# alevar/tiebrush

Hardware: AMD Instinct MI355X
Metric: input alignment records/sec collapsed (tiebrush) + bases/sec covered (tiecov) (higher is better)
Workload: dtype int64; 1 GPU; c3: 64 synthetic sorted BAMs x 5000000 100bp reads per GPU, --clip collapse + tiecov -c -j of the result; records_per_gpu=320000000, groups_out=25086541, parallelism=files-per-rank x1, ranks_seen=1, resident=SoA in HBM before the timed region, contexts=3

## Files before the change

### tiebrush_amd/csrc/collapse.hip

```cpp
#include <stdlib.h>

#include <chrono>

#include "dev_common.hpp"
#include "rx_w64.hpp"
#include "scan_op.hpp"
#include "strategy.hpp"
#include "tbk_internal.h"
#include "wgroup.h"

namespace {

struct EffKey {
  uint32_t khi_h, khi_l;
  int32_t kend;
  uint32_t flag_cnt;
};
struct EffOp {
  __device__ __forceinline__ EffKey operator()(const EffKey& a, const EffKey& b) const {
    uint64_t ak = ((uint64_t)a.khi_h << 32) | a.khi_l, bk = ((uint64_t)b.khi_h << 32) | b.khi_l;
    bool take_b = (b.flag_cnt >> 31) || bk > ak || (bk == ak && b.kend > a.kend);
    EffKey r;
    r.khi_h = take_b ? b.khi_h : a.khi_h;
    r.khi_l = take_b ? b.khi_l : a.khi_l;
    r.kend = take_b ? b.kend : a.kend;
    r.flag_cnt = ((a.flag_cnt | b.flag_cnt) & 0x80000000u) | ((a.flag_cnt + b.flag_cnt) & 0x7FFFFFFFu);
// ... 2359 lines not shown
  cnt[o] = cig_off[rep[o] + 1] - c0;
  cfirst[o] = c0;
}
__device__ __forceinline__ uint32_t g2c_key_ops(uint64_t k1) {
  const uint32_t shape = (uint32_t)k1;
  return shape == 0x80000000u ? 1u : ((shape >> 30) == 3u ? 3u : 0u);
}
__global__ void g2c_count_key_k(uint32_t ng, const uint64_t* __restrict__ key, const uint32_t* __restrict__ rep, const uint32_t* __restrict__ cig_off,
                                uint32_t* __restrict__ cnt, uint32_t* __restrict__ cfirst) {
  uint32_t o = blockIdx.x * blockDim.x + threadIdx.x;
  if (o >= ng) return;
  uint32_t n = g2c_key_ops(key[2 * (size_t)o + 1]);
  if (n == 0) {
    const uint32_t c0 = cig_off[rep[o]];
    n = cig_off[rep[o] + 1] - c0;
    cfirst[o] = c0;
  }
  cnt[o] = n;
}
struct G2cPrep {
  int32_t *start, *end, *yi;
  uint32_t *jcnt, *ridx;
  unsigned long long* sums;
};
__global__ __launch_bounds__(256) void g2c_gather_key_k(uint32_t ng, const uint64_t* __restrict__ key, const double* __restrict__ yc,
                                                        const int64_t* __restrict__ yx, const uint32_t* __restrict__ cfirst,
                                                        const uint32_t* __restrict__ cnt, const uint32_t* __restrict__ cig,
                                                        const uint32_t* __restrict__ ooff, uint32_t total, int32_t* __restrict__ o_tid,
                                                        int32_t* __restrict__ o_pos, uint8_t* __restrict__ o_strand, double* __restrict__ o_yc,
                                                        int64_t* __restrict__ o_yx, uint32_t* __restrict__ o_cig_off, uint32_t* __restrict__ o_cig,
                                                        G2cPrep P) {
  unsigned long long mb = 0, ay = 0, nji = 0;
  uint32_t eb = 0;
  for (uint32_t o = blockIdx.x * blockDim.x + threadIdx.x; o < ng; o += gridDim.x * blockDim.x) {
    const uint64_t k0 = key[2 * (size_t)o], k1 = key[2 * (size_t)o + 1];
    const int32_t tidv = (int32_t)(uint32_t)(k0 >> 33) - 1, posv = (int32_t)(uint32_t)((k0 >> 2) & 0x7FFFFFFFull) - 1;
    o_tid[o] = tidv;
    o_pos[o] = posv;
    const uint32_t sc = (uint32_t)k0 & 3u;
    o_strand[o] = sc == 0u ? (uint8_t)'+' : (sc == 1u ? (uint8_t)'-' : (uint8_t)'.');
    const double y0 = (double)(float)yc[o];
    o_yc[o] = y0;
    o_yx[o] = yx[o];
    const uint32_t d = ooff[o];
    o_cig_off[o] = d;
    if (o + 1 == ng) o_cig_off[ng] = total;
    const uint32_t shape = (uint32_t)k1, span = (uint32_t)(k1 >> 32);
    int l, nex = 0;
    if (shape == 0x80000000u) {
      o_cig[d] = (span << 4) | C_M;
      l = (int)span;
      nex = 1;
      mb += span;
    } else if ((shape >> 30) == 3u) {
      const uint32_t a = (shape >> 20) & 0x3FFu, g = shape & 0xFFFFFu;
      o_cig[d] = (a << 4) | C_M;
      o_cig[d + 1] = (g << 4) | C_N;
      o_cig[d + 2] = ((span - a - g) << 4) | C_M;
      l = (int)span;
      nex = 2;
      mb += span - g;
    } else {
      const uint32_t c0 = cfirst[o], n = cnt[o];
      l = walk_exons(posv, cig + c0, n, [](int, int) {}, &nex);
      for (uint32_t k = 0; k < n; ++k) {
        const uint32_t w = cig[c0 + k];
        o_cig[d + k] = w;
        const uint32_t op = cig_op(w);
        if (op == C_M)
          mb += cig_len(w);
        else if (op != C_I && op != C_D && op != C_N && op != C_S)
          eb |= TBK_DERR_FATALOP;
      }
      if (n >= 256) eb |= TBK_DERR_NCIGAR;
    }
    double y = y0;
    if (!(y == rint(y)) || !(fabs(y) < 1073741824.0)) {
      eb |= TBK_DERR_FRACTIONAL;
      y = 0.0;
    } else {
      ay += (unsigned long long)fabs(y);
    }
    P.ridx[o] = o;
    P.yi[o] = (int32_t)y;
    P.start[o] = posv + 1;
    P.end[o] = posv + l;
    P.jcnt[o] = (uint32_t)(nex - 1);
    nji += (unsigned long long)(nex - 1);
  }
  __shared__ unsigned long long red_mb[4], red_ay[4], red_nj[4];
  __shared__ uint32_t red_e[4];
  mb = wave_sum(mb);
  ay = wave_sum(ay);
  nji = wave_sum(nji);
#pragma unroll
  for (int dd = 32; dd >= 1; dd >>= 1) eb |= __shfl_xor(eb, dd, 64);
  if (lane_id() == 0) {
    red_mb[threadIdx.x >> 6] = mb;
    red_ay[threadIdx.x >> 6] = ay;
    red_nj[threadIdx.x >> 6] = nji;
    red_e[threadIdx.x >> 6] = eb;
  }
  __syncthreads();
  if (threadIdx.x == 0) {
    for (int q = 1; q < 4; ++q) {
      mb += red_mb[q];
      ay += red_ay[q];
      nji += red_nj[q];
      eb |= red_e[q];
    }
    if (mb) atomicAdd(&P.sums[0], mb);
    if (ay) atomicAdd(&P.sums[1], ay);
    if (eb) atomicOr(&P.sums[2], (unsigned long long)eb);
    if (nji) atomicAdd(&P.sums[3], nji);
  }
}
__global__ void g2c_gather_k(uint32_t ng, const uint32_t* __restrict__ rep, const double* __restrict__ yc, const int64_t* __restrict__ yx,
                             const int32_t* __restrict__ tid, const int32_t* __restrict__ pos, const uint8_t* __restrict__ strand,
                             const uint32_t* __restrict__ cfirst, const uint32_t* __restrict__ cnt, const uint32_t* __restrict__ cig,
                             const uint32_t* __restrict__ ooff, uint32_t total, int32_t* __restrict__ o_tid, int32_t* __restrict__ o_pos,
                             uint8_t* __restrict__ o_strand, double* __restrict__ o_yc, int64_t* __restrict__ o_yx,
                             uint32_t* __restrict__ o_cig_off, uint32_t* __restrict__ o_cig) {
  uint32_t o = blockIdx.x * blockDim.x + threadIdx.x;
  if (o >= ng) return;
  uint32_t r = rep[o];
  o_tid[o] = tid[r];
  o_pos[o] = pos[r];
  o_strand[o] = strand[r];
  o_yc[o] = (double)(float)yc[o];
  o_yx[o] = yx[o];
  uint32_t d = ooff[o];
  o_cig_off[o] = d;
  if (o + 1 == ng) o_cig_off[ng] = total;
  const uint32_t c0 = cfirst[o], n = cnt[o];
  for (uint32_t k = 0; k < n; ++k) o_cig[d + k] = cig[c0 + k];
}
}

// ... 17 lines not shown
int tbk_cov_view_build(tbk_ctx* ctx, const int32_t* r_tid, const int32_t* r_pos, const uint8_t* r_strand, const uint32_t* r_cig_off,
                       const uint32_t* r_cig, const uint32_t* g_rep, const double* g_yc, const int64_t* g_yx, uint32_t ng, tbk_cov_in* view,
                       const uint64_t* g_key) {
  memset(view, 0, sizeof(*view));
  view->mem = TBK_MEM_DEVICE;
  ctx->view_prep.valid = false;
  if (ng == 0) return 0;
  uint32_t* cnt = ws_alloc<uint32_t>(ctx, ng);
  uint32_t* ooff = ws_alloc<uint32_t>(ctx, ng);
  uint32_t* cfirst = ws_alloc<uint32_t>(ctx, ng);
  if (!cfirst) return TBK_ENOMEM;
  const uint32_t B = 256;
  if (g_key)
    TBK_LAUNCH(ctx, "g2c_count", g2c_count_key_k, cdiv(ng, B), B, 0, ng, g_key, g_rep, r_cig_off, cnt, cfirst);
  else
    TBK_LAUNCH(ctx, "g2c_count", g2c_count_k, cdiv(ng, B), B, 0, ng, g_rep, r_cig_off, cnt, cfirst);
  TBK_TRY(tbk_exscan_u32(ctx, cnt, ooff, ng, ctx->d_scalars + 20));
  TBK_HIP(hipMemcpyAsync(ctx->h_scalars + 20, ctx->d_scalars + 20, sizeof(uint64_t), hipMemcpyDeviceToHost, ctx->stream));
  TBK_HIP(hipStreamSynchronize(ctx->stream));
  const uint64_t total = ctx->h_scalars[20];
  if (total >= (1ull << 32)) return TBK_E2BIG;
  auto al = [](size_t x) { return (x + 255) & ~(size_t)255; };
  size_t need = al((size_t)ng * 4) * 2 + al(ng) + al((size_t)ng * 8) * 2 + al((size_t)(ng + 1) * 4) + al((size_t)total * 4 + 4) +
                (g_key ? al((size_t)ng * 4) * 5 : 0);
  if (need > ctx->d_view_cap) {
    if (ctx->d_view) (void)hipFree(ctx->d_view);
    ctx->d_view = nullptr;
    ctx->d_view_cap = 0;
    size_t cap = need + need / 4;
    TBK_HIP(hipMalloc((void**)&ctx->d_view, cap));
    ctx->d_view_cap = cap;
  }
  char* p = ctx->d_view;
  auto take = [&](size_t bytes) {
    char* r = p;
    p += al(bytes);
    return r;
  };
  int32_t* o_tid = (int32_t*)take((size_t)ng * 4);
  int32_t* o_pos = (int32_t*)take((size_t)ng * 4);
  uint8_t* o_strand = (uint8_t*)take(ng);
  double* o_yc = (double*)take((size_t)ng * 8);
  int64_t* o_yx = (int64_t*)take((size_t)ng * 8);
  uint32_t* o_cig_off = (uint32_t*)take((size_t)(ng + 1) * 4);
  uint32_t* o_cig = (uint32_t*)take((size_t)total * 4 + 4);
  G2cPrep P{};
  if (g_key) {
    P.start = (int32_t*)take((size_t)ng * 4);
    P.end = (int32_t*)take((size_t)ng * 4);
    P.yi = (int32_t*)take((size_t)ng * 4);
    P.jcnt = (uint32_t*)take((size_t)ng * 4);
    P.ridx = (uint32_t*)take((size_t)ng * 4);
    P.sums = (unsigned long long*)(ctx->d_scalars + 24);
    TBK_HIP(hipMemsetAsync(P.sums, 0, 4 * sizeof(uint64_t), ctx->stream));
    TBK_LAUNCH(ctx, "g2c_gather", g2c_gather_key_k, (cdiv(ng, B) < 4096u ? cdiv(ng, B) : 4096u), B, 0, ng, g_key, g_yc, g_yx, cfirst, cnt, r_cig, ooff,
               (uint32_t)total, o_tid, o_pos, o_strand, o_yc, o_yx, o_cig_off, o_cig, P);
    TBK_HIP(hipMemcpyAsync(ctx->h_scalars + 24, ctx->d_scalars + 24, 4 * sizeof(uint64_t), hipMemcpyDeviceToHost, ctx->stream));
  } else
    TBK_LAUNCH(ctx, "g2c_gather", g2c_gather_k, cdiv(ng, B), B, 0, ng, g_rep, g_yc, g_yx, r_tid, r_pos, r_strand, cfirst, cnt, r_cig, ooff,
               (uint32_t)total, o_tid, o_pos, o_strand, o_yc, o_yx, o_cig_off, o_cig);
  TBK_HIP(hipStreamSynchronize(ctx->stream));
  TBK_TRY(tbk_check_launch(ctx, "groups_to_cov_in"));
  view->n_records = ng;
  view->n_cigar_ops = (uint32_t)total;
  view->tid = o_tid;
  view->pos = o_pos;
  view->flag = nullptr;
  view->cig_off = o_cig_off;
  view->cig = o_cig;
  view->yc = o_yc;
  view->strand = o_strand;
  view->yx = o_yx;
  if (g_key) {
    auto& V = ctx->view_prep;
    V.cig = o_cig;
    V.n = ng;
    V.start = P.start;
    V.end = P.end;
    V.yi = P.yi;
    V.jcnt = P.jcnt;
    V.ridx = P.ridx;
    V.n_bases = ctx->h_scalars[24];
    V.sum_abs = ctx->h_scalars[25];
    V.err = (uint32_t)ctx->h_scalars[26];
    V.n_junc = ctx->h_scalars[27];
    V.valid = true;
  }
  return 0;
}
```

### tiebrush_amd/csrc/cov.hip

```cpp
#include <thread>

#include "dev_common.hpp"
#include "scan_op.hpp"
#include "tbk_internal.h"

namespace {

constexpr int COV_W = 8192;
constexpr int COV_NT = 256;
constexpr int COV_PER = COV_W / COV_NT;

struct SegMax {
  int32_t mx;
  uint32_t flag;
};
struct SegMaxOp {
  __device__ __forceinline__ SegMax operator()(const SegMax& a, const SegMax& b) const {
    SegMax r;
    r.mx = b.flag ? b.mx : (a.mx > b.mx ? a.mx : b.mx);
    r.flag = a.flag | b.flag;
    return r;
  }
};

// ... 109 lines not shown
};
struct BundleStore {
  CovArrays A;
  uint32_t m;
  uint64_t* nb_out;
  uint32_t* err;
  __device__ __forceinline__ void operator()(uint32_t j, const SegMax& v, const SegMax& inc, const SegMax&, uint32_t head, uint32_t before,
                                             const int2& a) const {
    const int32_t t = a.y, st = a.x;
    if (!v.flag && st < A.start[j - 1]) atomicOr(err, TBK_DERR_UNSORTED);
    const uint32_t b = before + head - 1u;
    A.bhead[j] = head;
    A.bid[j] = b;
    if (head) {
      A.b_tid[b] = t;
      A.b_start[b] = st;
    }
    const bool last = j + 1 == m;
    if (last || A.tid[j + 1] != t || A.start[j + 1] > inc.mx) A.b_end[b] = inc.mx;
    if (last) *nb_out = (uint64_t)b + 1u;
  }
};

struct CbAgg {
  int32_t first_tid, last_tid;
  int32_t mx;
  uint32_t whole;
};
struct CbOp {
  __device__ __forceinline__ CbAgg operator()(const CbAgg& a, const CbAgg& b) const {
    if (b.last_tid == INT32_MIN) return a;
    if (a.last_tid == INT32_MIN) return b;
    CbAgg r;
    r.first_tid = a.first_tid;
    r.last_tid = b.last_tid;
    const bool joins = b.whole && b.first_tid == a.last_tid;
    r.mx = joins ? (a.mx > b.mx ? a.mx : b.mx) : b.mx;
    r.whole = joins ? a.whole : 0u;
    return r;
  }
};
constexpr uint32_t CB_NT = 256, CB_ROWS = 4, CB_TILE = CB_NT * 4 * CB_ROWS;
__device__ __forceinline__ void cb_load4(const int32_t* __restrict__ a, uint64_t i, uint32_t m, int32_t fill, int32_t v[4]) {
  if (i + 3 < m) {
    const int4 q = *reinterpret_cast<const int4*>(a + i);
    v[0] = q.x, v[1] = q.y, v[2] = q.z, v[3] = q.w;
  } else {
#pragma unroll
    for (int e = 0; e < 4; ++e) v[e] = i + e < m ? a[i + e] : fill;
  }
}
template <class T, class Op>
__device__ __forceinline__ T wave_incl_scan_op(T v, Op op) {
#pragma unroll
  for (int d = 1; d < 64; d <<= 1) {
    const T o = shfl_up_t(v, d);
    if ((int)lane_id() >= d) v = op(o, v);
  }
  return v;
}
__device__ __forceinline__ void cb_put(uint64_t* p, uint64_t v) { __hip_atomic_store(p, v, __ATOMIC_RELAXED, __HIP_MEMORY_SCOPE_AGENT); }
__device__ __forceinline__ uint64_t cb_get(const uint64_t* p) { return __hip_atomic_load(p, __ATOMIC_RELAXED, __HIP_MEMORY_SCOPE_AGENT); }
__device__ __forceinline__ uint4 cb_get4(const uint4* p) {
  const uint64_t a = cb_get(reinterpret_cast<const uint64_t*>(p)), b = cb_get(reinterpret_cast<const uint64_t*>(p) + 1);
  return make_uint4((uint32_t)a, (uint32_t)(a >> 32), (uint32_t)b, (uint32_t)(b >> 32));
}
__device__ __forceinline__ bool cb_last_block(uint32_t* __restrict__ done) {
  __shared__ uint32_t s_last;
  if (threadIdx.x == 0) {
    __builtin_amdgcn_s_waitcnt(TBK_WAIT_VMCNT0);
    __asm__ volatile("" ::: "memory");
    s_last = atomicAdd(done, 1u) == gridDim.x - 1u ? 1u : 0u;
  }
  __syncthreads();
  return s_last != 0u;
}
template <uint32_t NT>
__device__ __forceinline__ void cb_spine_block(uint4* __restrict__ part, uint32_t ntiles, CbAgg* wl ) {
  const CbOp op{};
  const CbAgg none{0, INT32_MIN, INT32_MIN, 1u};
  auto un = [](const uint4& v) { return CbAgg{(int32_t)v.x, (int32_t)v.y, (int32_t)v.z, v.w}; };
  auto pk = [](const CbAgg& a) { return make_uint4((uint32_t)a.first_tid, (uint32_t)a.last_tid, (uint32_t)a.mx, a.whole); };
  const uint4 none4 = pk(none);
  const uint32_t per = (ntiles + NT - 1u) / NT, i0 = threadIdx.x * per, i1 = i0 + per < ntiles ? i0 + per : ntiles;
  CbAgg a = none;
  for (uint32_t q0 = i0; q0 < i1; q0 += 8u) {
    uint4 v8[8];
#pragma unroll
    for (uint32_t u = 0; u < 8u; ++u) v8[u] = q0 + u < i1 ? cb_get4(part + q0 + u) : none4;
#pragma unroll
    for (uint32_t u = 0; u < 8u; ++u) a = op(a, un(v8[u]));
  }
  const CbAgg inc = wave_incl_scan_op(a, op);
  if (lane_id() == 63) wl[threadIdx.x >> 6] = inc;
  CbAgg run = shfl_up_t(inc, 1);
  __syncthreads();
  {
    CbAgg acc = none;
    const uint32_t wv = threadIdx.x >> 6;
    for (uint32_t q = 0; q < wv; ++q) acc = op(acc, wl[q]);
    run = lane_id() == 0 ? acc : op(acc, run);
  }
  for (uint32_t q0 = i0; q0 < i1; q0 += 8u) {
    uint4 v8[8];
#pragma unroll
    for (uint32_t u = 0; u < 8u; ++u) v8[u] = q0 + u < i1 ? cb_get4(part + q0 + u) : none4;
#pragma unroll
    for (uint32_t u = 0; u < 8u; ++u) {
      if (q0 + u < i1) part[q0 + u] = pk(run);
      run = op(run, un(v8[u]));
    }
  }
}
__global__ __launch_bounds__(CB_NT) void cb_agg_k(uint32_t m, const int32_t* __restrict__ tid, const int32_t* __restrict__ end, uint4* __restrict__ part,
                                                  uint32_t* __restrict__ done) {
  constexpr uint32_t NWV = CB_NT / 64;
  __shared__ CbAgg wl[CB_ROWS * NWV];
  const CbOp op{};
  const CbAgg none{0, INT32_MIN, INT32_MIN, 1u};
  int32_t t4[CB_ROWS][4], e4[CB_ROWS][4];
#pragma unroll
  for (uint32_t r = 0; r < CB_ROWS; ++r) {
    const uint64_t i = (uint64_t)blockIdx.x * CB_TILE + ((uint64_t)r * CB_NT + threadIdx.x) * 4u;
    cb_load4(tid, i, m, 0, t4[r]);
    cb_load4(end, i, m, 0, e4[r]);
  }
#pragma unroll
  for (uint32_t r = 0; r < CB_ROWS; ++r) {
    const uint64_t i = (uint64_t)blockIdx.x * CB_TILE + ((uint64_t)r * CB_NT + threadIdx.x) * 4u;
    CbAgg a = none;
#pragma unroll
    for (int e = 0; e < 4; ++e)
      if (i + e < m) a = op(a, CbAgg{t4[r][e], t4[r][e], e4[r][e], 1u});
    a = wave_incl_scan_op(a, op);
    if (lane_id() == 63) wl[r * NWV + (threadIdx.x >> 6)] = a;
  }
  __syncthreads();
  if (threadIdx.x == 0) {
    CbAgg run = none;
#pragma unroll
    for (uint32_t q = 0; q < CB_ROWS * NWV; ++q) run = op(run, wl[q]);
    uint64_t* o = reinterpret_cast<uint64_t*>(part + blockIdx.x);
    cb_put(o, (uint64_t)(uint32_t)run.first_tid | ((uint64_t)(uint32_t)run.last_tid << 32));
    cb_put(o + 1, (uint64_t)(uint32_t)run.mx | ((uint64_t)run.whole << 32));
  }
  if (cb_last_block(done)) cb_spine_block<CB_NT>(part, gridDim.x, wl);
}
template <bool EMIT>
__global__ __launch_bounds__(CB_NT) void cb_heads_k(uint32_t m, CovArrays A, const uint4* __restrict__ part, uint32_t* __restrict__ hcnt,
                                                    const uint32_t* __restrict__ hbase, uint64_t* __restrict__ nb_out, uint32_t* __restrict__ err) {
  __shared__ CbAgg sm[CB_NT / 64];
  __shared__ uint32_t smu[8];
  const CbOp op{};
  const CbAgg none{0, INT32_MIN, INT32_MIN, 1u};
  const uint4 pv = part[blockIdx.x];
  CbAgg run{(int32_t)pv.x, (int32_t)pv.y, (int32_t)pv.z, pv.w};
  uint32_t heads_tile = 0, hrun = EMIT ? hbase[blockIdx.x] : 0u;
  bool bad = false;
#pragma unroll
  for (uint32_t r = 0; r < CB_ROWS; ++r) {
    const uint64_t i = (uint64_t)blockIdx.x * CB_TILE + ((uint64_t)r * CB_NT + threadIdx.x) * 4u;
    int32_t t4[4], s4[4], e4[4];
    cb_load4(A.tid, i, m, 0, t4);
    cb_load4(A.start, i, m, 0, s4);
    cb_load4(A.end, i, m, 0, e4);
    CbAgg a = none;
#pragma unroll
// ... 1459 lines not shown
    TBK_LAUNCH(ctx, "junc_write", junc_write_k, cdiv(nj, B), B, 0, nj, A, sb.hi, sb.lo, sb.val, head, hoff, in->yc, out->cap_junctions,
               out->j_tid, out->j_start, out->j_end, out->j_strand, out->j_val);
  }
  TBK_HIP(hipMemcpyAsync(ctx->h_scalars + 9, sc + 9, sizeof(uint64_t), hipMemcpyDeviceToHost, ctx->stream));
  TBK_HIP(hipStreamSynchronize(ctx->stream));
  *nju_out = (uint32_t)ctx->h_scalars[9];
  return tbk_check_launch(ctx, "junctions");
}

struct JuncSide {
  TbkWorker* w = nullptr;
  bool th = false;
  int rc = 0;
  int join() {
    if (th) {
      w->wait();
      th = false;
    }
    return rc;
  }
  ~JuncSide() { (void)join(); }
};

static int cov_intervals_lean(tbk_ctx* ctx, const tbk_cov_in* in, tbk_cov_out* out, CovArrays A, uint32_t m, bool all_valid, uint64_t sum_abs) {
  const uint32_t B = 256;
  uint64_t* sc = ctx->d_scalars;
  const uint32_t cbt = cdiv(m, CB_TILE);
  uint4* cpart = ws_alloc<uint4>(ctx, cbt);
  uint32_t* hcnt = ws_alloc<uint32_t>(ctx, cbt);
  uint32_t* hbase = ws_alloc<uint32_t>(ctx, cbt);
  long long* xsum = ws_alloc<long long>(ctx, cbt);
  long long* xbase = ws_alloc<long long>(ctx, cbt);
  ClChunks L;
  L.base = ws_alloc<uint32_t>(ctx, cbt);
  L.cnt = ws_alloc<uint32_t>(ctx, cbt);
  L.tbase = ws_alloc<uint32_t>(ctx, cbt);
  L.j = ws_alloc<uint32_t>(ctx, m);
  L.cs = ws_alloc<uint64_t>(ctx, m);
  ClTiles T;
  uint64_t cap64 = (uint64_t)m / 8u > (1ull << 20) ? (uint64_t)m / 8u : (1ull << 20);
  if (ctx->dbg.cov_tile_cap) cap64 = ctx->dbg.cov_tile_cap;
  T.cap = (uint32_t)cap64;
  T.first = ws_alloc<uint32_t>(ctx, (size_t)T.cap + 1);
  T.tb = ws_alloc<uint32_t>(ctx, (size_t)T.cap + 1);
  T.cnt = ws_alloc<uint32_t>(ctx, (size_t)T.cap + 1);
  if (!cpart || !hcnt || !hbase || !xsum || !xbase || !L.base || !L.cnt || !L.tbase || !L.j || !L.cs || !T.first || !T.tb || !T.cnt) return TBK_ENOMEM;
  TBK_HIP(hipMemsetAsync(T.cnt, 0, ((size_t)T.cap + 1) * 4, ctx->stream));
  uint32_t* done = (uint32_t*)(sc + 16);
  TBK_HIP(hipMemsetAsync(done, 0, sizeof(uint64_t), ctx->stream));
  TBK_LAUNCH(ctx, "cov_bundles", cb_agg_k, cbt, CB_NT, 0, m, A.tid, A.end, cpart, done);
  TBK_LAUNCH(ctx, "cov_bundles", cl_heads_k<false>, cbt, CB_NT, 0, m, A, cpart, hcnt, xsum, (const uint32_t*)nullptr, (const long long*)nullptr, in->cig_off,
             in->cig, T, L, sc, ctx->d_err, done + 1, hbase, xbase);
  TBK_LAUNCH(ctx, "cov_place", cl_heads_k<true>, cbt, CB_NT, 0, m, A, cpart, hcnt, xsum, hbase, xbase, in->cig_off, in->cig, T, L, sc, ctx->d_err,
             (uint32_t*)nullptr, (uint32_t*)nullptr, (long long*)nullptr);
  uint32_t eb = 0;
  TBK_TRY(tbk_sync_err(ctx, &eb));
  if (eb) return tbk_derr_to_status(ctx, eb);
  if (ctx->h_scalars[CL_SC_REFUSED]) return 1;
  const uint32_t nb = (uint32_t)ctx->h_scalars[CL_SC_NB];
  const uint64_t S = ctx->h_scalars[CL_SC_S], nspill = ctx->h_scalars[CL_SC_NSPILL];
  const uint32_t nsl = (uint32_t)ctx->h_scalars[CL_SC_NSL];
  out->span_bases = S;
  const uint32_t ntiles = (uint32_t)((S + COV_W - 1) / COV_W);
  if (nspill >= (1ull << 32)) return TBK_E2BIG;
  const uint64_t cp_cap64 = 2ull * ((uint64_t)in->n_cigar_ops + nspill) + nb + ntiles + 16;
  if (cp_cap64 >= (1ull << 32)) return TBK_E2BIG;
  const uint32_t cp_cap = (uint32_t)cp_cap64;
  uint32_t* tile_off = ws_alloc<uint32_t>(ctx, (size_t)ntiles + 1);
  uint32_t* tile_fill = ws_alloc<uint32_t>(ctx, (size_t)ntiles + 1);
  uint32_t* sp_seg = ws_alloc<uint32_t>(ctx, nspill + 1);
  uint32_t* sp_rec = ws_alloc<uint32_t>(ctx, nspill + 1);
  uint64_t* cp_pos = ws_alloc<uint64_t>(ctx, cp_cap);
  double* cp_val = ws_alloc<double>(ctx, cp_cap);
  uint32_t* tile_cp_base = ws_alloc<uint32_t>(ctx, ntiles);
  uint32_t* tile_cp_cnt = ws_alloc<uint32_t>(ctx, ntiles);
  uint32_t* icnt = ws_alloc<uint32_t>(ctx, ntiles);
// ... 96 lines not shown
  out->n_bases = ctx->h_scalars[0];
  const uint64_t sum_abs = ctx->h_scalars[1];
  const bool integral = !fractional && !sample_mode && sum_abs < (1ull << 52);
  const uint64_t nj_known = prepared ? V.n_junc : (want_j ? ctx->h_scalars[14] : ~0ull);
  if (m == 0) return 0;
  if (want_j && want_cov && m >= COV_SIDE_MIN) {
    tbk_ctx* jc = tbk_side_ctx(ctx);
    if (jc) {
      const size_t hint = (size_t)m * 8 + (size_t)in->n_cigar_ops * 64 + ((size_t)4 << 20);
      if (!ctx->side_worker) ctx->side_worker = new TbkWorker();
      side.w = ctx->side_worker;
      side.th = true;
      side.w->post([&side, jc, hint, m, &A, in, jcnt, out, integral, nj_known, &nj, &nju]() {
        side.rc = tbk_side_begin(jc, hint);
        if (side.rc == 0) side.rc = junc_branch(jc, m, A, in, jcnt, out, integral, nj_known, &nj, &nju);
        tbk_side_end(jc);
      });
    }
  }

  bool lean_done = false;
  if (want_cov && !fractional && !sample_mode && !ctx->dbg.cov_legacy && !ctx->dbg.cov_bundle_scan) {
    const size_t ws_mark = ctx->ws_off;
    const int lrc = cov_intervals_lean(ctx, in, out, A, m, all_valid, sum_abs);
    if (lrc < 0) return lrc;
    lean_done = lrc == 0;
    if (!lean_done) {
      if (ctx->ws_overflow.empty()) ctx->ws_off = ws_mark;
      TBK_HIP(hipMemsetAsync(sc + 3, 0, 11 * sizeof(uint64_t), ctx->stream));
    }
  }
  if (!lean_done) {
  {
    if (ctx->dbg.cov_bundle_scan) {
      BundleLoad ld{A.tid, A.end};
      BundleAux ax{A.tid, A.start};
      BundleHead hd{};
      BundleStore st{A, m, sc + 3, ctx->d_err};
      SegMax ident{INT32_MIN, 0u};
      TBK_TRY((scan_two_run<4, SegMax, SegMaxOp, uint32_t, SoPlusU32, BundleLoad, BundleAux, BundleHead, BundleStore>(ctx, "cov_bundles", m, ld, ax, hd, st, SegMaxOp{}, ident,
                                                                                                          SoPlusU32{}, 0u)));
    } else {
      const uint32_t cbt = cdiv(m, CB_TILE);
      uint4* cpart = ws_alloc<uint4>(ctx, cbt);
      uint32_t* hcnt = ws_alloc<uint32_t>(ctx, cbt);
      uint32_t* hbase = ws_alloc<uint32_t>(ctx, cbt);
      if (!cpart || !hcnt || !hbase) return TBK_ENOMEM;
// ... 143 lines not shown
```

### tiebrush_amd/csrc/tbk_api.hip

```cpp
#include <sys/mman.h>

#include <algorithm>
#include <chrono>
#include <mutex>
#include <vector>
#include <new>

#include "tbk_internal.h"

namespace {
std::mutex g_reg_m;
struct RegEntry {
  void* p;
  int users;
};
std::vector<RegEntry> g_reg;
}

static void release_registered(tbk_ctx* ctx) {
  if (ctx->registered.empty()) return;
  (void)hipStreamSynchronize(ctx->stream);
  const auto r0 = std::chrono::steady_clock::now();
  struct RP {
    tbk_ctx* c;
// ... 431 lines not shown
    if (end == std::string::npos) end = s.size();
    const std::string kv = s.substr(at, end - at);
    at = end + 1;
    const size_t eq = kv.find('=');
    const std::string k = kv.substr(0, eq), v = eq == std::string::npos ? std::string("1") : kv.substr(eq + 1);
    const unsigned long long u = strtoull(v.c_str(), nullptr, 0);
    const bool on = v != "0";
    if (k == "path") out->path = v == "sort" ? 1 : (v == "window" ? 2 : 0);
    else if (k == "raw") out->raw = on ? 1 : 0;
    else if (k == "sort") out->sort = v == "radix" ? 1 : (v == "runs" ? 2 : 0);
    else if (k == "scan") out->scan = v == "lookback" ? 1 : (v == "3pass" ? 2 : 0);
    else if (k == "hash_mask") out->hash_mask = (uint32_t)u;
    else if (k == "qhash_mask") out->qhash_mask = u;
    else if (k == "yd_wave_min") out->yd_wave_min = (uint32_t)u;
    else if (k == "yd_bgrid") out->yd_bgrid = (uint32_t)u;
    else if (k == "yd_radix") out->yd_radix = on;
    else if (k == "yd_literal") out->yd_literal = on;
    else if (k == "yd_own_arena") out->yd_own_arena = on;
    else if (k == "wg_dense_verify") out->wg_dense_verify = on;
    else if (k == "wg_rank_merge") out->wg_rank_merge = on;
    else if (k == "cov_legacy") out->cov_legacy = on;
    else if (k == "cov_bundle_scan") out->cov_bundle_scan = on;
    else if (k == "cov_prep") out->cov_prep = on;
    else if (k == "cov_tile_cap") out->cov_tile_cap = u;
    else if (k == "junc_radix") out->junc_radix = on;
    else if (k == "no_junc_agg") out->no_junc_agg = on;
    else if (k == "jh_cap") out->jh_cap = (uint32_t)u;
    else if (k == "index_chain") out->index_chain = on;
    else if (k == "no_register") out->no_register = on;
    else if (k == "phases") out->phases = on;
    else if (k == "no_bounce") out->no_bounce = on;
    else if (k == "fmt_slice") out->fmt_slice = u;
  }
}

extern "C" {

int tbk_abi_version(void) { return TBK_ABI_VERSION; }

int tbk_set_debug(tbk_ctx* ctx, const char* spec) {
  if (!ctx) return TBK_EINVAL;
  tbk_debug_parse(spec, &ctx->dbg);
  if (ctx->yd_ctx) ctx->yd_ctx->dbg = ctx->dbg;
  if (ctx->side_ctx) ctx->side_ctx->dbg = ctx->dbg;
  return 0;
}
// ... 494 lines not shown
```

### tiebrush_amd/csrc/tbk_internal.h

```cpp
#pragma once
#include <hip/hip_runtime.h>
#include <stdint.h>
#include <stdio.h>
#include <string.h>

#include <string>
#include <condition_variable>
#include <functional>
#include <mutex>
#include <thread>
#include <utility>
#include <vector>

#include "../../include/tbk.h"

enum : uint32_t {
  TBK_DERR_UNSORTED = 1u << 0,
  TBK_DERR_COLLISION = 1u << 1,
  TBK_DERR_FATALOP = 1u << 2,
  TBK_DERR_SPAN = 1u << 3,
  TBK_DERR_NCIGAR = 1u << 4,
  TBK_DERR_FRACTIONAL = 1u << 5,
  TBK_DERR_OVERFLOW = 1u << 6,
  TBK_DERR_INTERNAL = 1u << 7,
// ... 45 lines not shown
    {
      std::lock_guard<std::mutex> lk(m);
      quit = true;
    }
    cv.notify_all();
    if (th.joinable()) th.join();
  }
};

struct TbkDebug {
  int path = 0;
  int raw = -1;
  int sort = 0;
  int scan = 0;
  uint32_t hash_mask = 0xFFFFFFFFu;
  uint64_t qhash_mask = ~0ull;
  uint32_t yd_wave_min = 0;
  uint32_t yd_bgrid = 0;
  bool yd_radix = false;
  bool yd_literal = false;
  bool yd_own_arena = false;
  bool wg_dense_verify = false, wg_rank_merge = false;
  bool cov_legacy = false, cov_bundle_scan = false, cov_prep = false, junc_radix = false, no_junc_agg = false;
  uint64_t cov_tile_cap = 0;
  uint32_t jh_cap = 0;
  bool index_chain = false;
  bool no_register = false;
  bool no_bounce = false;
  bool phases = false;
  uint64_t fmt_slice = 0;
};
void tbk_debug_parse(const char* spec, TbkDebug* out);

struct tbk_ctx {
  int device = 0;
  TbkDebug dbg;
  hipStream_t own_stream = nullptr;
  hipStream_t stream = nullptr;
  hipStream_t aux = nullptr;
  hipEvent_t aux_done = nullptr;
  char* ws = nullptr;
  size_t ws_cap = 0, ws_off = 0;
  size_t ws_top = 0;
  bool ws_top_mode = false;
  bool ws_borrowed = false;
  std::vector<std::pair<char*, size_t>> ws_overflow;
  size_t ws_over_used = 0;
  uint32_t* d_err = nullptr;
  uint64_t* d_scalars = nullptr;
  uint64_t* h_scalars = nullptr;
  hipEvent_t stage_ev = nullptr;
  char* d_view = nullptr;
  size_t d_view_cap = 0;
  struct ViewPrep {
    bool valid = false;
    const void* cig = nullptr;
    uint32_t n = 0;
    int32_t *start = nullptr, *end = nullptr, *yi = nullptr;
    uint32_t *jcnt = nullptr, *ridx = nullptr;
    uint64_t n_bases = 0, sum_abs = 0, n_junc = 0;
    uint32_t err = 0;
  } view_prep;
  bool profiling = false;
  std::vector<KTime> ktimes;
  std::vector<hipEvent_t> ev_pool;
  size_t ev_used = 0;
  std::vector<tbk_kernel_time> last_times;
  std::string last_error;
  int num_cu = 256;
  void* yd_job = nullptr;
  tbk_ctx* yd_ctx = nullptr;
  TbkWorker* yd_worker = nullptr;
  bool yd_pending = false;
  int yd_rc = 0;
  size_t ws_base_off = 0;
  tbk_ctx* side_ctx = nullptr;
  TbkWorker* side_worker = nullptr;
  bool side_times_pending = false;
  std::vector<void*> registered;
  char* d_unpack = nullptr;
  size_t d_unpack_cap = 0;
  std::vector<uint8_t> unpack_tbm;
// ... 121 lines not shown
```

Before: 20.24 billion records/s.

## Fuse coverage bundle aggregation and spine scan into the group-to-collapse gather kernel

After: 20.23 billion records/s. About the same (-0.0%).

```diff
diff --git a/tiebrush_amd/csrc/collapse.hip b/tiebrush_amd/csrc/collapse.hip
--- a/tiebrush_amd/csrc/collapse.hip
+++ b/tiebrush_amd/csrc/collapse.hip
@@ -2,6 +2,7 @@
 
 #include <chrono>
 
+#include "cov_agg.hpp"
 #include "dev_common.hpp"
 #include "rx_w64.hpp"
 #include "scan_op.hpp"
@@ -2407,71 +2408,149 @@
   int32_t *start, *end, *yi;
   uint32_t *jcnt, *ridx;
   unsigned long long* sums;
+  uint4* cpart;
+  uint32_t* done;
 };
-__global__ __launch_bounds__(256) void g2c_gather_key_k(uint32_t ng, const uint64_t* __restrict__ key, const double* __restrict__ yc,
-                                                        const int64_t* __restrict__ yx, const uint32_t* __restrict__ cfirst,
-                                                        const uint32_t* __restrict__ cnt, const uint32_t* __restrict__ cig,
-                                                        const uint32_t* __restrict__ ooff, uint32_t total, int32_t* __restrict__ o_tid,
-                                                        int32_t* __restrict__ o_pos, uint8_t* __restrict__ o_strand, double* __restrict__ o_yc,
-                                                        int64_t* __restrict__ o_yx, uint32_t* __restrict__ o_cig_off, uint32_t* __restrict__ o_cig,
-                                                        G2cPrep P) {
+__global__ __launch_bounds__(CB_NT) void g2c_gather_key_k(uint32_t ng, const uint64_t* __restrict__ key, const double* __restrict__ yc,
+                                                          const int64_t* __restrict__ yx, const uint32_t* __restrict__ cfirst,
+                                                          const uint32_t* __restrict__ cnt, const uint32_t* __restrict__ cig,
+                                                          const uint32_t* __restrict__ ooff, uint32_t total, int32_t* __restrict__ o_tid,
+                                                          int32_t* __restrict__ o_pos, uint8_t* __restrict__ o_strand, double* __restrict__ o_yc,
+                                                          int64_t* __restrict__ o_yx, uint32_t* __restrict__ o_cig_off, uint32_t* __restrict__ o_cig,
+                                                          G2cPrep P) {
+  constexpr uint32_t NWV = CB_NT / 64;
+  __shared__ CbAgg wl[2][CB_ROWS * NWV];
+  const CbOp op{};
+  const CbAgg none{0, INT32_MIN, INT32_MIN, 1u};
+  const uint32_t ntiles = (uint32_t)(((uint64_t)ng + CB_TILE - 1u) / CB_TILE);
   unsigned long long mb = 0, ay = 0, nji = 0;
-  uint32_t eb = 0;
-  for (uint32_t o = blockIdx.x * blockDim.x + threadIdx.x; o < ng; o += gridDim.x * blockDim.x) {
-    const uint64_t k0 = key[2 * (size_t)o], k1 = key[2 * (size_t)o + 1];
-    const int32_t tidv = (int32_t)(uint32_t)(k0 >> 33) - 1, posv = (int32_t)(uint32_t)((k0 >> 2) & 0x7FFFFFFFull) - 1;
-    o_tid[o] = tidv;
-    o_pos[o] = posv;
-    const uint32_t sc = (uint32_t)k0 & 3u;
-    o_strand[o] = sc == 0u ? (uint8_t)'+' : (sc == 1u ? (uint8_t)'-' : (uint8_t)'.');
-    const double y0 = (double)(float)yc[o];
-    o_yc[o] = y0;
-    o_yx[o] = yx[o];
-    const uint32_t d = ooff[o];
-    o_cig_off[o] = d;
-    if (o + 1 == ng) o_cig_off[ng] = total;
-    const uint32_t shape = (uint32_t)k1, span = (uint32_t)(k1 >> 32);
-    int l, nex = 0;
-    if (shape == 0x80000000u) {
-      o_cig[d] = (span << 4) | C_M;
-      l = (int)span;
-      nex = 1;
-      mb += span;
-    } else if ((shape >> 30) == 3u) {
-      const uint32_t a = (shape >> 20) & 0x3FFu, g = shape & 0xFFFFFu;
-      o_cig[d] = (a << 4) | C_M;
-      o_cig[d + 1] = (g << 4) | C_N;
-      o_cig[d + 2] = ((span - a - g) << 4) | C_M;
-      l = (int)span;
-      nex = 2;
-      mb += span - g;
-    } else {
-      const uint32_t c0 = cfirst[o], n = cnt[o];
-      l = walk_exons(posv, cig + c0, n, [](int, int) {}, &nex);
-      for (uint32_t k = 0; k < n; ++k) {
-        const uint32_t w = cig[c0 + k];
-        o_cig[d + k] = w;
-        const uint32_t op = cig_op(w);
-        if (op == C_M)
-          mb += cig_len(w);
-        else if (op != C_I && op != C_D && op != C_N && op != C_S)
-          eb |= TBK_DERR_FATALOP;
-      }
-      if (n >= 256) eb |= TBK_DERR_NCIGAR;
-    }
-    double y = y0;
-    if (!(y == rint(y)) || !(fabs(y) < 1073741824.0)) {
-      eb |= TBK_DERR_FRACTIONAL;
-      y = 0.0;
-    } else {
-      ay += (unsigned long long)fabs(y);
-    }
-    P.ridx[o] = o;
-    P.yi[o] = (int32_t)y;
-    P.start[o] = posv + 1;
-    P.end[o] = posv + l;
-    P.jcnt[o] = (uint32_t)(nex - 1);
-    nji += (unsigned long long)(nex - 1);
+  uint32_t eb = 0, par = 0;
+  for (uint32_t tile = blockIdx.x; tile < ntiles; tile += gridDim.x, par ^= 1u) {
+#pragma unroll 1
+    for (uint32_t r = 0; r < CB_ROWS; ++r) {
+      const uint64_t i0 = (uint64_t)tile * CB_TILE + ((uint64_t)r * CB_NT + threadIdx.x) * 4u;
+      const uint32_t nv = i0 < ng ? ((uint64_t)ng - i0 < 4u ? (uint32_t)(ng - i0) : 4u) : 0u;
+      CbAgg a = none;
+      if (nv) {
+        uint64_t k0[4], k1[4];
+        double y0[4];
+        int64_t x0[4];
+        uint32_t d[4];
+#pragma unroll
+        for (uint32_t e = 0; e < 4u; ++e) {
+          const size_t o = (size_t)i0 + (e < nv ? e : 0u);
+          k0[e] = key[2 * o], k1[e] = key[2 * o + 1];
+          y0[e] = (double)(float)yc[o];
+          x0[e] = yx[o];
+          d[e] = ooff[o];
+        }
+        int32_t tidv[4], posv[4], len[4], yi[4];
+        uint32_t strand = 0, c0[4], n[4], jc[4];
+#pragma unroll
+        for (uint32_t e = 0; e < 4u; ++e) {
+          tidv[e] = (int32_t)(uint32_t)(k0[e] >> 33) - 1, posv[e] = (int32_t)(uint32_t)((k0[e] >> 2) & 0x7FFFFFFFull) - 1;
+          const uint32_t sc = (uint32_t)k0[e] & 3u;
+          strand |= (sc == 0u ? (uint32_t)'+' : (sc == 1u ? (uint32_t)'-' : (uint32_t)'.')) << (8u * e);
+          const uint32_t shape = (uint32_t)k1[e], span = (uint32_t)(k1[e] >> 32);
+          int nex;
+          c0[e] = 0, n[e] = 0;
+          if (shape == 0x80000000u) {
+            len[e] = (int)span;
+            nex = 1;
+            if (e < nv) mb += span;
+          } else if ((shape >> 30) == 3u) {
+            len[e] = (int)span;
+            nex = 2;
+            if (e < nv) mb += span - (shape & 0xFFFFFu);
+          } else if (e < nv) {
+            c0[e] = cfirst[i0 + e], n[e] = cnt[i0 + e];
+            len[e] = walk_exons(posv[e], cig + c0[e], n[e], [](int, int) {}, &nex);
+            if (n[e] >= 256) eb |= TBK_DERR_NCIGAR;
+          } else {
+            len[e] = 0;
+            nex = 1;
+          }
+          jc[e] = (uint32_t)(nex - 1);
+          double y = y0[e];
+          if (!(y == rint(y)) || !(fabs(y) < 1073741824.0)) {
+            if (e < nv) eb |= TBK_DERR_FRACTIONAL;
+            y = 0.0;
+          } else if (e < nv) {
+            ay += (unsigned long long)fabs(y);
+          }
+          yi[e] = (int32_t)y;
+          if (e < nv) {
+            nji += (unsigned long long)jc[e];
+            a = op(a, CbAgg{tidv[e], tidv[e], posv[e] + len[e], 1u});
+          }
+        }
+#pragma unroll
+        for (uint32_t e = 0; e < 4u; ++e) {
+          if (e >= nv) break;
+          const uint32_t shape = (uint32_t)k1[e], span = (uint32_t)(k1[e] >> 32);
+          if (shape == 0x80000000u) {
+            o_cig[d[e]] = (span << 4) | C_M;
+          } else if ((shape >> 30) == 3u) {
+            const uint32_t ma = (shape >> 20) & 0x3FFu, g = shape & 0xFFFFFu;
+            o_cig[d[e]] = (ma << 4) | C_M;
+            o_cig[d[e] + 1] = (g << 4) | C_N;
+            o_cig[d[e] + 2] = ((span - ma - g) << 4) | C_M;
+          } else {
+            for (uint32_t k = 0; k < n[e]; ++k) {
+              const uint32_t w = cig[c0[e] + k];
+              o_cig[d[e] + k] = w;
+              const uint32_t cop = cig_op(w);
+              if (cop == C_M)
+                mb += cig_len(w);
+              else if (cop != C_I && cop != C_D && cop != C_N && cop != C_S)
+                eb |= TBK_DERR_FATALOP;
+            }
+          }
+        }
+        if (nv == 4u) {
+          *reinterpret_cast<int4*>(o_tid + i0) = make_int4(tidv[0], tidv[1], tidv[2], tidv[3]);
+          *reinterpret_cast<int4*>(o_pos + i0) = make_int4(posv[0], posv[1], posv[2], posv[3]);
+          *reinterpret_cast<uint32_t*>(o_strand + i0) = strand;
+          *reinterpret_cast<double2*>(o_yc + i0) = make_double2(y0[0], y0[1]);
+          *reinterpret_cast<double2*>(o_yc + i0 + 2) = make_double2(y0[2], y0[3]);
+          *reinterpret_cast<longlong2*>(o_yx + i0) = make_longlong2(x0[0], x0[1]);
+          *reinterpret_cast<longlong2*>(o_yx + i0 + 2) = make_longlong2(x0[2], x0[3]);
+          *reinterpret_cast<uint4*>(o_cig_off + i0) = make_uint4(d[0], d[1], d[2], d[3]);
+          *reinterpret_cast<uint4*>(P.ridx + i0) = make_uint4((uint32_t)i0, (uint32_t)i0 + 1u, (uint32_t)i0 + 2u, (uint32_t)i0 + 3u);
+          *reinterpret_cast<int4*>(P.yi + i0) = make_int4(yi[0], yi[1], yi[2], yi[3]);
+          *reinterpret_cast<int4*>(P.start + i0) = make_int4(posv[0] + 1, posv[1] + 1, posv[2] + 1, posv[3] + 1);
+          *reinterpret_cast<int4*>(P.end + i0) = make_int4(posv[0] + len[0], posv[1] + len[1], posv[2] + len[2], posv[3] + len[3]);
+          *reinterpret_cast<uint4*>(P.jcnt + i0) = make_uint4(jc[0], jc[1], jc[2], jc[3]);
+        } else {
+#pragma unroll
+          for (uint32_t e = 0; e < 3u; ++e) {
+            if (e >= nv) break;
+            const size_t o = (size_t)i0 + e;
+            o_tid[o] = tidv[e];
+            o_pos[o] = posv[e];
+            o_strand[o] = (uint8_t)(strand >> (8u * e));
+            o_yc[o] = y0[e];
+            o_yx[o] = x0[e];
+            o_cig_off[o] = d[e];
+            P.ridx[o] = (uint32_t)o;
+            P.yi[o] = yi[e];
+            P.start[o] = posv[e] + 1;
+            P.end[o] = posv[e] + len[e];
+            P.jcnt[o] = jc[e];
+          }
+        }
+        if (i0 + nv == ng) o_cig_off[ng] = total;
+      }
+      a = wave_incl_scan_op(a, op);
+      if (lane_id() == 63) wl[par][r * NWV + (threadIdx.x >> 6)] = a;
+    }
+    __syncthreads();
+    if (threadIdx.x == 0) {
+      CbAgg run = none;
+#pragma unroll
+      for (uint32_t q = 0; q < CB_ROWS * NWV; ++q) run = op(run, wl[par][q]);
+      cb_put_agg(P.cpart + tile, run);
+    }
   }
   __shared__ unsigned long long red_mb[4], red_ay[4], red_nj[4];
   __shared__ uint32_t red_e[4];
@@ -2499,6 +2578,7 @@
     if (eb) atomicOr(&P.sums[2], (unsigned long long)eb);
     if (nji) atomicAdd(&P.sums[3], nji);
   }
+  if (cb_last_block(P.done)) cb_spine_block<CB_NT>(P.cpart, ntiles, wl[0]);
 }
 __global__ void g2c_gather_k(uint32_t ng, const uint32_t* __restrict__ rep, const double* __restrict__ yc, const int64_t* __restrict__ yx,
                              const int32_t* __restrict__ tid, const int32_t* __restrict__ pos, const uint8_t* __restrict__ strand,
@@ -2562,7 +2642,7 @@
   if (total >= (1ull << 32)) return TBK_E2BIG;
   auto al = [](size_t x) { return (x + 255) & ~(size_t)255; };
   size_t need = al((size_t)ng * 4) * 2 + al(ng) + al((size_t)ng * 8) * 2 + al((size_t)(ng + 1) * 4) + al((size_t)total * 4 + 4) +
-                (g_key ? al((size_t)ng * 4) * 5 : 0);
+                (g_key ? al((size_t)ng * 4) * 5 + al((size_t)cdiv(ng, CB_TILE) * sizeof(uint4)) : 0);
   if (need > ctx->d_view_cap) {
     if (ctx->d_view) (void)hipFree(ctx->d_view);
     ctx->d_view = nullptr;
@@ -2591,10 +2671,15 @@
     P.yi = (int32_t*)take((size_t)ng * 4);
     P.jcnt = (uint32_t*)take((size_t)ng * 4);
     P.ridx = (uint32_t*)take((size_t)ng * 4);
+    const uint32_t cbt = cdiv(ng, CB_TILE);
+    P.cpart = (uint4*)take((size_t)cbt * sizeof(uint4));
     P.sums = (unsigned long long*)(ctx->d_scalars + 24);
-    TBK_HIP(hipMemsetAsync(P.sums, 0, 4 * sizeof(uint64_t), ctx->stream));
-    TBK_LAUNCH(ctx, "g2c_gather", g2c_gather_key_k, (cdiv(ng, B) < 4096u ? cdiv(ng, B) : 4096u), B, 0, ng, g_key, g_yc, g_yx, cfirst, cnt, r_cig, ooff,
-               (uint32_t)total, o_tid, o_pos, o_strand, o_yc, o_yx, o_cig_off, o_cig, P);
+    P.done = (uint32_t*)(ctx->d_scalars + 29);
+    TBK_HIP(hipMemsetAsync(P.sums, 0, 6 * sizeof(uint64_t), ctx->stream));
+    uint32_t grid = cbt < 4096u ? cbt : 4096u;
+    if (ctx->dbg.g2c_grid && ctx->dbg.g2c_grid < grid) grid = ctx->dbg.g2c_grid;
+    TBK_LAUNCH(ctx, "g2c_gather", g2c_gather_key_k, grid, CB_NT, 0, ng, g_key, g_yc, g_yx, cfirst, cnt, r_cig, ooff, (uint32_t)total, o_tid, o_pos,
+               o_strand, o_yc, o_yx, o_cig_off, o_cig, P);
     TBK_HIP(hipMemcpyAsync(ctx->h_scalars + 24, ctx->d_scalars + 24, 4 * sizeof(uint64_t), hipMemcpyDeviceToHost, ctx->stream));
   } else
     TBK_LAUNCH(ctx, "g2c_gather", g2c_gather_k, cdiv(ng, B), B, 0, ng, g_rep, g_yc, g_yx, r_tid, r_pos, r_strand, cfirst, cnt, r_cig, ooff,
@@ -2620,6 +2705,9 @@
     V.yi = P.yi;
     V.jcnt = P.jcnt;
     V.ridx = P.ridx;
+    V.cpart = P.cpart;
+    V.ctiles = cdiv(ng, CB_TILE);
+    V.ctile = CB_TILE;
     V.n_bases = ctx->h_scalars[24];
     V.sum_abs = ctx->h_scalars[25];
     V.err = (uint32_t)ctx->h_scalars[26];
diff --git a/tiebrush_amd/csrc/cov.hip b/tiebrush_amd/csrc/cov.hip
--- a/tiebrush_amd/csrc/cov.hip
+++ b/tiebrush_amd/csrc/cov.hip
@@ -1,5 +1,6 @@
 #include <thread>
 
+#include "cov_agg.hpp"
 #include "dev_common.hpp"
 #include "scan_op.hpp"
 #include "tbk_internal.h"
@@ -155,25 +156,6 @@
   }
 };
 
-struct CbAgg {
-  int32_t first_tid, last_tid;
-  int32_t mx;
-  uint32_t whole;
-};
-struct CbOp {
-  __device__ __forceinline__ CbAgg operator()(const CbAgg& a, const CbAgg& b) const {
-    if (b.last_tid == INT32_MIN) return a;
-    if (a.last_tid == INT32_MIN) return b;
-    CbAgg r;
-    r.first_tid = a.first_tid;
-    r.last_tid = b.last_tid;
-    const bool joins = b.whole && b.first_tid == a.last_tid;
-    r.mx = joins ? (a.mx > b.mx ? a.mx : b.mx) : b.mx;
-    r.whole = joins ? a.whole : 0u;
-    return r;
-  }
-};
-constexpr uint32_t CB_NT = 256, CB_ROWS = 4, CB_TILE = CB_NT * 4 * CB_ROWS;
 __device__ __forceinline__ void cb_load4(const int32_t* __restrict__ a, uint64_t i, uint32_t m, int32_t fill, int32_t v[4]) {
   if (i + 3 < m) {
     const int4 q = *reinterpret_cast<const int4*>(a + i);
@@ -181,68 +163,6 @@
   } else {
 #pragma unroll
     for (int e = 0; e < 4; ++e) v[e] = i + e < m ? a[i + e] : fill;
-  }
-}
-template <class T, class Op>
-__device__ __forceinline__ T wave_incl_scan_op(T v, Op op) {
-#pragma unroll
-  for (int d = 1; d < 64; d <<= 1) {
-    const T o = shfl_up_t(v, d);
-    if ((int)lane_id() >= d) v = op(o, v);
-  }
-  return v;
-}
-__device__ __forceinline__ void cb_put(uint64_t* p, uint64_t v) { __hip_atomic_store(p, v, __ATOMIC_RELAXED, __HIP_MEMORY_SCOPE_AGENT); }
-__device__ __forceinline__ uint64_t cb_get(const uint64_t* p) { return __hip_atomic_load(p, __ATOMIC_RELAXED, __HIP_MEMORY_SCOPE_AGENT); }
-__device__ __forceinline__ uint4 cb_get4(const uint4* p) {
-  const uint64_t a = cb_get(reinterpret_cast<const uint64_t*>(p)), b = cb_get(reinterpret_cast<const uint64_t*>(p) + 1);
-  return make_uint4((uint32_t)a, (uint32_t)(a >> 32), (uint32_t)b, (uint32_t)(b >> 32));
-}
-__device__ __forceinline__ bool cb_last_block(uint32_t* __restrict__ done) {
-  __shared__ uint32_t s_last;
-  if (threadIdx.x == 0) {
-    __builtin_amdgcn_s_waitcnt(TBK_WAIT_VMCNT0);
-    __asm__ volatile("" ::: "memory");
-    s_last = atomicAdd(done, 1u) == gridDim.x - 1u ? 1u : 0u;
-  }
-  __syncthreads();
-  return s_last != 0u;
-}
-template <uint32_t NT>
-__device__ __forceinline__ void cb_spine_block(uint4* __restrict__ part, uint32_t ntiles, CbAgg* wl ) {
-  const CbOp op{};
-  const CbAgg none{0, INT32_MIN, INT32_MIN, 1u};
-  auto un = [](const uint4& v) { return CbAgg{(int32_t)v.x, (int32_t)v.y, (int32_t)v.z, v.w}; };
-  auto pk = [](const CbAgg& a) { return make_uint4((uint32_t)a.first_tid, (uint32_t)a.last_tid, (uint32_t)a.mx, a.whole); };
-  const uint4 none4 = pk(none);
-  const uint32_t per = (ntiles + NT - 1u) / NT, i0 = threadIdx.x * per, i1 = i0 + per < ntiles ? i0 + per : ntiles;
-  CbAgg a = none;
-  for (uint32_t q0 = i0; q0 < i1; q0 += 8u) {
-    uint4 v8[8];
-#pragma unroll
-    for (uint32_t u = 0; u < 8u; ++u) v8[u] = q0 + u < i1 ? cb_get4(part + q0 + u) : none4;
-#pragma unroll
-    for (uint32_t u = 0; u < 8u; ++u) a = op(a, un(v8[u]));
-  }
-  const CbAgg inc = wave_incl_scan_op(a, op);
-  if (lane_id() == 63) wl[threadIdx.x >> 6] = inc;
-  CbAgg run = shfl_up_t(inc, 1);
-  __syncthreads();
-  {
-    CbAgg acc = none;
-    const uint32_t wv = threadIdx.x >> 6;
-    for (uint32_t q = 0; q < wv; ++q) acc = op(acc, wl[q]);
-    run = lane_id() == 0 ? acc : op(acc, run);
-  }
-  for (uint32_t q0 = i0; q0 < i1; q0 += 8u) {
-    uint4 v8[8];
-#pragma unroll
-    for (uint32_t u = 0; u < 8u; ++u) v8[u] = q0 + u < i1 ? cb_get4(part + q0 + u) : none4;
-#pragma unroll
-    for (uint32_t u = 0; u < 8u; ++u) {
-      if (q0 + u < i1) part[q0 + u] = pk(run);
-      run = op(run, un(v8[u]));
-    }
   }
 }
 __global__ __launch_bounds__(CB_NT) void cb_agg_k(uint32_t m, const int32_t* __restrict__ tid, const int32_t* __restrict__ end, uint4* __restrict__ part,
@@ -273,9 +193,7 @@
     CbAgg run = none;
 #pragma unroll
     for (uint32_t q = 0; q < CB_ROWS * NWV; ++q) run = op(run, wl[q]);
-    uint64_t* o = reinterpret_cast<uint64_t*>(part + blockIdx.x);
-    cb_put(o, (uint64_t)(uint32_t)run.first_tid | ((uint64_t)(uint32_t)run.last_tid << 32));
-    cb_put(o + 1, (uint64_t)(uint32_t)run.mx | ((uint64_t)run.whole << 32));
+    cb_put_agg(part + blockIdx.x, run);
   }
   if (cb_last_block(done)) cb_spine_block<CB_NT>(part, gridDim.x, wl);
 }
@@ -1781,11 +1699,12 @@
   ~JuncSide() { (void)join(); }
 };
 
-static int cov_intervals_lean(tbk_ctx* ctx, const tbk_cov_in* in, tbk_cov_out* out, CovArrays A, uint32_t m, bool all_valid, uint64_t sum_abs) {
+static int cov_intervals_lean(tbk_ctx* ctx, const tbk_cov_in* in, tbk_cov_out* out, CovArrays A, uint32_t m, bool all_valid, uint64_t sum_abs,
+                              const uint4* spine) {
   const uint32_t B = 256;
   uint64_t* sc = ctx->d_scalars;
   const uint32_t cbt = cdiv(m, CB_TILE);
-  uint4* cpart = ws_alloc<uint4>(ctx, cbt);
+  uint4* cpart = spine ? nullptr : ws_alloc<uint4>(ctx, cbt);
   uint32_t* hcnt = ws_alloc<uint32_t>(ctx, cbt);
   uint32_t* hbase = ws_alloc<uint32_t>(ctx, cbt);
   long long* xsum = ws_alloc<long long>(ctx, cbt);
@@ -1803,14 +1722,17 @@
   T.first = ws_alloc<uint32_t>(ctx, (size_t)T.cap + 1);
   T.tb = ws_alloc<uint32_t>(ctx, (size_t)T.cap + 1);
   T.cnt = ws_alloc<uint32_t>(ctx, (size_t)T.cap + 1);
-  if (!cpart || !hcnt || !hbase || !xsum || !xbase || !L.base || !L.cnt || !L.tbase || !L.j || !L.cs || !T.first || !T.tb || !T.cnt) return TBK_ENOMEM;
+  if ((!spine && !cpart) || !hcnt || !hbase || !xsum || !xbase || !L.base || !L.cnt || !L.tbase || !L.j || !L.cs || !T.first || !T.tb || !T.cnt) return TBK_ENOMEM;
   TBK_HIP(hipMemsetAsync(T.cnt, 0, ((size_t)T.cap + 1) * 4, ctx->stream));
   uint32_t* done = (uint32_t*)(sc + 16);
   TBK_HIP(hipMemsetAsync(done, 0, sizeof(uint64_t), ctx->stream));
-  TBK_LAUNCH(ctx, "cov_bundles", cb_agg_k, cbt, CB_NT, 0, m, A.tid, A.end, cpart, done);
-  TBK_LAUNCH(ctx, "cov_bundles", cl_heads_k<false>, cbt, CB_NT, 0, m, A, cpart, hcnt, xsum, (const uint32_t*)nullptr, (const long long*)nullptr, in->cig_off,
+  if (!spine) {
+    TBK_LAUNCH(ctx, "cov_bundles", cb_agg_k, cbt, CB_NT, 0, m, A.tid, A.end, cpart, done);
+    spine = cpart;
+  }
+  TBK_LAUNCH(ctx, "cov_bundles", cl_heads_k<false>, cbt, CB_NT, 0, m, A, spine, hcnt, xsum, (const uint32_t*)nullptr, (const long long*)nullptr, in->cig_off,
              in->cig, T, L, sc, ctx->d_err, done + 1, hbase, xbase);
-  TBK_LAUNCH(ctx, "cov_place", cl_heads_k<true>, cbt, CB_NT, 0, m, A, cpart, hcnt, xsum, hbase, xbase, in->cig_off, in->cig, T, L, sc, ctx->d_err,
+  TBK_LAUNCH(ctx, "cov_place", cl_heads_k<true>, cbt, CB_NT, 0, m, A, spine, hcnt, xsum, hbase, xbase, in->cig_off, in->cig, T, L, sc, ctx->d_err,
              (uint32_t*)nullptr, (uint32_t*)nullptr, (long long*)nullptr);
   uint32_t eb = 0;
   TBK_TRY(tbk_sync_err(ctx, &eb));
@@ -1953,7 +1875,8 @@
   bool lean_done = false;
   if (want_cov && !fractional && !sample_mode && !ctx->dbg.cov_legacy && !ctx->dbg.cov_bundle_scan) {
     const size_t ws_mark = ctx->ws_off;
-    const int lrc = cov_intervals_lean(ctx, in, out, A, m, all_valid, sum_abs);
+    const bool spined = prepared && V.cpart && V.ctile == CB_TILE && V.ctiles == cdiv(m, CB_TILE) && !ctx->dbg.cov_agg;
+    const int lrc = cov_intervals_lean(ctx, in, out, A, m, all_valid, sum_abs, spined ? (const uint4*)V.cpart : nullptr);
     if (lrc < 0) return lrc;
     lean_done = lrc == 0;
     if (!lean_done) {
diff --git a/tiebrush_amd/csrc/cov_agg.hpp b/tiebrush_amd/csrc/cov_agg.hpp
--- /dev/null
+++ b/tiebrush_amd/csrc/cov_agg.hpp
@@ -0,0 +1,90 @@
+#pragma once
+#include "dev_common.hpp"
+#include "scan_op.hpp"
+
+struct CbAgg {
+  int32_t first_tid, last_tid;
+  int32_t mx;
+  uint32_t whole;
+};
+struct CbOp {
+  __device__ __forceinline__ CbAgg operator()(const CbAgg& a, const CbAgg& b) const {
+    if (b.last_tid == INT32_MIN) return a;
+    if (a.last_tid == INT32_MIN) return b;
+    CbAgg r;
+    r.first_tid = a.first_tid;
+    r.last_tid = b.last_tid;
+    const bool joins = b.whole && b.first_tid == a.last_tid;
+    r.mx = joins ? (a.mx > b.mx ? a.mx : b.mx) : b.mx;
+    r.whole = joins ? a.whole : 0u;
+    return r;
+  }
+};
+constexpr uint32_t CB_NT = 256, CB_ROWS = 4, CB_TILE = CB_NT * 4 * CB_ROWS;
+template <class T, class Op>
+__device__ __forceinline__ T wave_incl_scan_op(T v, Op op) {
+#pragma unroll
+  for (int d = 1; d < 64; d <<= 1) {
+    const T o = shfl_up_t(v, d);
+    if ((int)lane_id() >= d) v = op(o, v);
+  }
+  return v;
+}
+__device__ __forceinline__ void cb_put(uint64_t* p, uint64_t v) { __hip_atomic_store(p, v, __ATOMIC_RELAXED, __HIP_MEMORY_SCOPE_AGENT); }
+__device__ __forceinline__ uint64_t cb_get(const uint64_t* p) { return __hip_atomic_load(p, __ATOMIC_RELAXED, __HIP_MEMORY_SCOPE_AGENT); }
+__device__ __forceinline__ uint4 cb_get4(const uint4* p) {
+  const uint64_t a = cb_get(reinterpret_cast<const uint64_t*>(p)), b = cb_get(reinterpret_cast<const uint64_t*>(p) + 1);
+  return make_uint4((uint32_t)a, (uint32_t)(a >> 32), (uint32_t)b, (uint32_t)(b >> 32));
+}
+__device__ __forceinline__ void cb_put_agg(uint4* p, const CbAgg& a) {
+  uint64_t* o = reinterpret_cast<uint64_t*>(p);
+  cb_put(o, (uint64_t)(uint32_t)a.first_tid | ((uint64_t)(uint32_t)a.last_tid << 32));
+  cb_put(o + 1, (uint64_t)(uint32_t)a.mx | ((uint64_t)a.whole << 32));
+}
+__device__ __forceinline__ bool cb_last_block(uint32_t* __restrict__ done) {
+  __shared__ uint32_t s_last;
+  if (threadIdx.x == 0) {
+    __builtin_amdgcn_s_waitcnt(TBK_WAIT_VMCNT0);
+    __asm__ volatile("" ::: "memory");
+    s_last = atomicAdd(done, 1u) == gridDim.x - 1u ? 1u : 0u;
+  }
+  __syncthreads();
+  return s_last != 0u;
+}
+template <uint32_t NT>
+__device__ __forceinline__ void cb_spine_block(uint4* __restrict__ part, uint32_t ntiles, CbAgg* wl ) {
+  const CbOp op{};
+  const CbAgg none{0, INT32_MIN, INT32_MIN, 1u};
+  auto un = [](const uint4& v) { return CbAgg{(int32_t)v.x, (int32_t)v.y, (int32_t)v.z, v.w}; };
+  auto pk = [](const CbAgg& a) { return make_uint4((uint32_t)a.first_tid, (uint32_t)a.last_tid, (uint32_t)a.mx, a.whole); };
+  const uint4 none4 = pk(none);
+  const uint32_t per = (ntiles + NT - 1u) / NT, i0 = threadIdx.x * per, i1 = i0 + per < ntiles ? i0 + per : ntiles;
+  CbAgg a = none;
+  for (uint32_t q0 = i0; q0 < i1; q0 += 8u) {
+    uint4 v8[8];
+#pragma unroll
+    for (uint32_t u = 0; u < 8u; ++u) v8[u] = q0 + u < i1 ? cb_get4(part + q0 + u) : none4;
+#pragma unroll
+    for (uint32_t u = 0; u < 8u; ++u) a = op(a, un(v8[u]));
+  }
+  const CbAgg inc = wave_incl_scan_op(a, op);
+  if (lane_id() == 63) wl[threadIdx.x >> 6] = inc;
+  CbAgg run = shfl_up_t(inc, 1);
+  __syncthreads();
+  {
+    CbAgg acc = none;
+    const uint32_t wv = threadIdx.x >> 6;
+    for (uint32_t q = 0; q < wv; ++q) acc = op(acc, wl[q]);
+    run = lane_id() == 0 ? acc : op(acc, run);
+  }
+  for (uint32_t q0 = i0; q0 < i1; q0 += 8u) {
+    uint4 v8[8];
+#pragma unroll
+    for (uint32_t u = 0; u < 8u; ++u) v8[u] = q0 + u < i1 ? cb_get4(part + q0 + u) : none4;
+#pragma unroll
+    for (uint32_t u = 0; u < 8u; ++u) {
+      if (q0 + u < i1) part[q0 + u] = pk(run);
+      run = op(run, un(v8[u]));
+    }
+  }
+}
diff --git a/tiebrush_amd/csrc/tbk_api.hip b/tiebrush_amd/csrc/tbk_api.hip
--- a/tiebrush_amd/csrc/tbk_api.hip
+++ b/tiebrush_amd/csrc/tbk_api.hip
@@ -477,6 +477,8 @@
     else if (k == "cov_legacy") out->cov_legacy = on;
     else if (k == "cov_bundle_scan") out->cov_bundle_scan = on;
     else if (k == "cov_prep") out->cov_prep = on;
+    else if (k == "cov_agg") out->cov_agg = on;
+    else if (k == "g2c_grid") out->g2c_grid = (uint32_t)u;
     else if (k == "cov_tile_cap") out->cov_tile_cap = u;
     else if (k == "junc_radix") out->junc_radix = on;
     else if (k == "no_junc_agg") out->no_junc_agg = on;
diff --git a/tiebrush_amd/csrc/tbk_internal.h b/tiebrush_amd/csrc/tbk_internal.h
--- a/tiebrush_amd/csrc/tbk_internal.h
+++ b/tiebrush_amd/csrc/tbk_internal.h
@@ -91,6 +91,8 @@
   bool yd_own_arena = false;
   bool wg_dense_verify = false, wg_rank_merge = false;
   bool cov_legacy = false, cov_bundle_scan = false, cov_prep = false, junc_radix = false, no_junc_agg = false;
+  bool cov_agg = false;
+  uint32_t g2c_grid = 0;
   uint64_t cov_tile_cap = 0;
   uint32_t jh_cap = 0;
   bool index_chain = false;
@@ -127,6 +129,8 @@
     uint32_t n = 0;
     int32_t *start = nullptr, *end = nullptr, *yi = nullptr;
     uint32_t *jcnt = nullptr, *ridx = nullptr;
+    void* cpart = nullptr;
+    uint32_t ctiles = 0, ctile = 0;
     uint64_t n_bases = 0, sum_abs = 0, n_junc = 0;
     uint32_t err = 0;
   } view_prep;
```
